# codeandkey/kami

Hardware: AMD Instinct MI355X
Metric: NN leaf-evals/sec at batch 512 (119×8×8 planes), 1/2/4/8 MI355X (higher is better)
Workload: dtype bf16

## Files before the change

kami_amd/csrc/tower8_mfma.hip:

```cpp
#include "tower_common.h"

#include <atomic>

namespace kh {

using f32x4_t = float __attribute__((ext_vector_type(4)));
__device__ __forceinline__ void store_wt(f32x4_t* p, f32x4_t v) { asm volatile("global_store_dwordx4 %0, %1, off sc1" ::"v"(p), "v"(v) : "memory"); }
__device__ __forceinline__ void store_wt(float* p, float v) { asm volatile("global_store_dword %0, %1, off sc1" ::"v"(p), "v"(v) : "memory"); }

constexpr int T8_LAG = 1;
struct CPipe { unsigned ring; int cslot; };

__device__ __forceinline__ unsigned cpipe_advance(CPipe& p)
{
    p.cslot = (p.cslot + 1 == RING_D) ? 0 : p.cslot + 1;
    return p.ring + p.cslot * CHUNK;
}

__device__ __forceinline__ unsigned cpipe_step(CPipe& p)
{
    asm volatile("s_barrier" ::: "memory");
    __builtin_amdgcn_sched_barrier(0);
    p.cslot = (p.cslot + 1 == RING_D) ? 0 : p.cslot + 1;
    return p.ring + p.cslot * CHUNK;
}

__device__ __forceinline__ void pipe_issue4(Pipe& p, int hw, int lane)
{
    const char* sbase = p.stream + (size_t)p.next * CHUNK + hw * 4096;
    const unsigned dst = p.ring + p.islot * CHUNK + hw * 4096;
    const unsigned voff = lane * 16;
    unsigned keep;
    asm volatile("s_mov_b32 %0, m0\n\ts_mov_b32 m0, %3\n\ts_nop 0\n\t"
                 "global_load_lds_dwordx4 %1, %2\n\tglobal_load_lds_dwordx4 %1, %2 offset:1024\n\t"
                 "global_load_lds_dwordx4 %1, %2 offset:2048\n\tglobal_load_lds_dwordx4 %1, %2 offset:3072\n\t"
                 "s_mov_b32 m0, %0"
                 : "=&s"(keep) : "v"(voff), "s"(sbase), "s"(dst) : "memory");
    p.next = (p.next + 1 == p.nch) ? 0 : p.next + 1;
    p.islot = (p.islot + 1 == RING_D) ? 0 : p.islot + 1;
}

template <int VMX>
__device__ __forceinline__ void hpipe_step(Pipe& p, int hw, int lane)
{
    asm volatile("s_waitcnt vmcnt(%0)" ::"n"(4 * (RING_D - 3 - T8_LAG) + VMX) : "memory");
    asm volatile("s_barrier" ::: "memory");
    pipe_issue4(p, hw, lane);
}

template <typename T, int TAPS, int KS, int MS, int PAR, int NREG = 0, bool CF = false, int TAILV = 0>
__device__ __forceinline__ void gemm8_layer(CPipe& p, const char* smem, int lane, unsigned b_base, int stride,
                                            f32x16 (&acc)[MS], typename Elem<T>::vec8 (&A)[2][8],
                                            const typename Elem<T>::vec8* breg = nullptr)
{
    using V = typename Elem<T>::vec8;
    using S = LayerShape<TAPS, KS, MS>;
    constexpr int KPC = S::KPC;
    constexpr int NF = KPC * MS;
    V B[2][KPC];
#pragma unroll
    for (int k = 0; k < KPC; ++k) {
        if (k < NREG) B[PAR][k] = breg[k];
        else B[PAR][k] = *reinterpret_cast<const V*>(smem + b_base + b_offset<TAPS, KS, CF>(k, stride));
    }
#pragma unroll
    for (int n = 0; n < S::NCH; ++n) {
        const int cur = (PAR + n) & 1, nxt = cur ^ 1;
        const unsigned a_off = cpipe_step(p) + lane * 16;
#pragma unroll
        for (int f = 0; f < 8; ++f)
            if (n + 1 == S::NCH || f < NF) A[nxt][f] = *reinterpret_cast<const V*>(smem + a_off + f * 1024);
        if (n + 1 < S::NCH) {
#pragma unroll
            for (int k = 0; k < KPC; ++k) {
                if ((n + 1) * KPC + k < NREG) B[nxt][k] = breg[(n + 1) * KPC + k];
                else B[nxt][k] = *reinterpret_cast<const V*>(smem + b_base + b_offset<TAPS, KS, CF>((n + 1) * KPC + k, stride));
            }
        }
        if (TAILV > 0 && n == S::NCH - 1) {
#pragma unroll
            for (int ms = 0; ms < MS; ++ms)
#pragma unroll
                for (int k = 0; k < KPC; ++k) acc[ms] = Elem<T>::mfma(A[cur][k * MS + ms], B[cur][k], acc[ms]);
#pragma unroll
            for (int i = 0; i < KPC; ++i) {
                __builtin_amdgcn_sched_group_barrier(0x100, 2, 0);
                __builtin_amdgcn_sched_group_barrier(0x008, 1, 0);
            }
#pragma unroll
            for (int i = 0; i < (MS - 1) * KPC; ++i) {
                __builtin_amdgcn_sched_group_barrier(0x008, 1, 0);
                if (i > 0) __builtin_amdgcn_sched_group_barrier(0x002, TAILV, 0);
            }
            continue;
        }
#pragma unroll
        for (int k = 0; k < KPC; ++k)
#pragma unroll
            for (int ms = 0; ms < MS; ++ms) acc[ms] = Elem<T>::mfma(A[cur][k * MS + ms], B[cur][k], acc[ms]);
#pragma unroll
        for (int i = 0; i < NF; ++i) {
            __builtin_amdgcn_sched_group_barrier(0x100, 2, 0);
            __builtin_amdgcn_sched_group_barrier(0x008, 1, 0);
        }
    }
}

template <typename T, int PAR>
__device__ __forceinline__ void gemm8_dummy(CPipe& p, const char* smem, int lane, typename Elem<T>::vec8 (&A)[2][8])
{
    using V = typename Elem<T>::vec8;
    const unsigned a_off = cpipe_step(p) + lane * 16;
#pragma unroll
    for (int f = 0; f < 8; ++f) A[PAR ^ 1][f] = *reinterpret_cast<const V*>(smem + a_off + f * 1024);
}


enum { BM_RASTER = 0, BM_CENTRE = 1, BM_QUARTERS = 2 };
template <int TAPS, int KS, int BM>
__device__ __forceinline__ constexpr unsigned b_off8(int kk, int stride)
{
    if constexpr (BM == BM_QUARTERS) {
        const int pass = kk / (TAPS * KS / 4), k = kk % (TAPS * KS / 4);
        return b_offset<TAPS, KS / 4, false>(k, stride) + pass * (KS / 4) * 32;
    }
    return b_offset<TAPS, KS, BM == BM_CENTRE>(kk, stride);
}

template <typename T, int TAPS, int KS, int MS, int PAR, int NREG, int BM, int N0, int N1, bool BARMID = false>
__device__ __forceinline__ void gemm8_steps(CPipe& p, const char* smem, int lane, unsigned b_base, int stride,
                                            f32x16 (&acc)[MS], typename Elem<T>::vec8 (&A)[2][8],
                                            typename Elem<T>::vec8 (&B)[2][8 / MS],
                                            const typename Elem<T>::vec8* breg = nullptr)
{
    using V = typename Elem<T>::vec8;
    using S = LayerShape<TAPS, KS, MS>;
    constexpr int KPC = S::KPC;
#pragma unroll
    for (int n = N0; n < N1; ++n) {
        const int cur = (PAR + n) & 1, nxt = cur ^ 1;
        if (BARMID && n == N0) {
            static_assert(!BARMID || (MS == 2 && KPC == 4), "mid-step barrier: 2 x 4 chunk");
            const unsigned a_off = cpipe_advance(p) + lane * 16;
#pragma unroll
            for (int k = 0; k < 2; ++k) {
#pragma unroll
                for (int ms = 0; ms < 2; ++ms) {
                    const int i = 2 * k + ms;
                    A[nxt][2 * i] = *reinterpret_cast<const V*>(smem + a_off + (2 * i) * 1024);
                    A[nxt][2 * i + 1] = *reinterpret_cast<const V*>(smem + a_off + (2 * i + 1) * 1024);
                    acc[ms] = Elem<T>::mfma(A[cur][k * MS + ms], B[cur][k], acc[ms]);
                    __builtin_amdgcn_sched_barrier(0);
                }
            }
            asm volatile("s_barrier" ::: "memory");
#pragma unroll
            for (int k = 2; k < 4; ++k) {
#pragma unroll
                for (int ms = 0; ms < 2; ++ms) {
                    if (k == 2 && n + 1 < S::NCH) {
#pragma unroll
                        for (int j = 0; j < 2; ++j) {
                            const int kk = 2 * ms + j;
                            if ((n + 1) * KPC + kk < NREG) B[nxt][kk] = breg[(n + 1) * KPC + kk];
                            else B[nxt][kk] = *reinterpret_cast<const V*>(smem + b_base + b_off8<TAPS, KS, BM>((n + 1) * KPC + kk, stride));
                        }
                    }
                    acc[ms] = Elem<T>::mfma(A[cur][k * MS + ms], B[cur][k], acc[ms]);
                    __builtin_amdgcn_sched_barrier(0);
                }
            }
            continue;
        }
        const unsigned a_off = cpipe_step(p) + lane * 16;
#pragma unroll
        for (int f = 0; f < 8; ++f) A[nxt][f] = *reinterpret_cast<const V*>(smem + a_off + f * 1024);
        if (n + 1 < S::NCH) {
#pragma unroll
            for (int k = 0; k < KPC; ++k) {
                if ((n + 1) * KPC + k < NREG) B[nxt][k] = breg[(n + 1) * KPC + k];
                else B[nxt][k] = *reinterpret_cast<const V*>(smem + b_base + b_off8<TAPS, KS, BM>((n + 1) * KPC + k, stride));
            }
        }
#pragma unroll
        for (int k = 0; k < KPC; ++k)
#pragma unroll
            for (int ms = 0; ms < MS; ++ms) acc[ms] = Elem<T>::mfma(A[cur][k * MS + ms], B[cur][k], acc[ms]);
#pragma unroll
        for (int i = 0; i < 8; ++i) {
            __builtin_amdgcn_sched_group_barrier(0x100, 2, 0);
            __builtin_amdgcn_sched_group_barrier(0x008, 1, 0);
        }
    }
}

enum { EPI_STEM = 0, EPI_PACK = 1, EPI_RESID = 2 };

template <typename T, int EPI, int G>
__device__ __forceinline__ u32x2 epi_group(const f32x16& acc, f32x16& xf)
{
    u32x2 o;
    if (EPI == EPI_PACK) {
        o.x = relu_pk(pack2<T>(acc[4 * G + 0], acc[4 * G + 1]));
        o.y = relu_pk(pack2<T>(acc[4 * G + 2], acc[4 * G + 3]));
    } else {
#pragma unroll
        for (int i = 0; i < 4; ++i) {
            const float t = relu_nan(acc[4 * G + i]);
            xf[4 * G + i] = EPI == EPI_RESID ? xf[4 * G + i] + t : t;
        }
        o.x = pack2<T>(xf[4 * G + 0], xf[4 * G + 1]);
        o.y = pack2<T>(xf[4 * G + 2], xf[4 * G + 3]);
    }
    return o;
}

#define T8_FENCE() __builtin_amdgcn_sched_barrier(0)

template <typename T, int EPI, int CURP>
__device__ __forceinline__ void boundary(CPipe& p, char* smem, int lane, f32x16 (&acc)[2], f32x16 (&nacc)[2],
                                         unsigned nshift, typename Elem<T>::vec8 (&A)[2][8],
                                         typename Elem<T>::vec8 (&B)[2][4], f32x16 (&xf)[2], unsigned out_pix, unsigned nb_base)
{
    using V = typename Elem<T>::vec8;
    constexpr int cur = CURP, nxt = CURP ^ 1;
    u32x2 o[2][4];
#define T8_LDN(ms, g) do { const float4 s_ = *reinterpret_cast<const float4*>(smem + nshift + ((ms) * 32 + 8 * (g)) * 4); \
        nacc[ms][4 * (g) + 0] = s_.x; nacc[ms][4 * (g) + 1] = s_.y; nacc[ms][4 * (g) + 2] = s_.z; nacc[ms][4 * (g) + 3] = s_.w; } while (0)
#define T8_ST(t, g) (*reinterpret_cast<u32x2*>(smem + out_pix + ((t) * 32 + 8 * (g)) * 2) = o[t][g])
#define T8_FRAG(ks) __builtin_bit_cast(V, (u32x4){ o[(ks) >> 1][2 * ((ks) & 1)].x, o[(ks) >> 1][2 * ((ks) & 1)].y, \
                                                   o[(ks) >> 1][2 * ((ks) & 1) + 1].x, o[(ks) >> 1][2 * ((ks) & 1) + 1].y })
    const unsigned a_off = cpipe_step(p) + lane * 16;
#define T8_RDA(set, f, off) (A[set][f] = *reinterpret_cast<const V*>(smem + (off) + (f) * 1024))
    T8_LDN(0, 0); T8_LDN(0, 1); acc[0] = Elem<T>::mfma(A[cur][0], B[cur][0], acc[0]); T8_FENCE();
    T8_LDN(0, 2); T8_LDN(0, 3); acc[0] = Elem<T>::mfma(A[cur][2], B[cur][1], acc[0]); T8_FENCE();
    T8_LDN(1, 0); T8_LDN(1, 1); acc[0] = Elem<T>::mfma(A[cur][4], B[cur][2], acc[0]); T8_FENCE();
    T8_LDN(1, 2); T8_LDN(1, 3); acc[0] = Elem<T>::mfma(A[cur][6], B[cur][3], acc[0]); T8_FENCE();
    T8_RDA(nxt, 0, a_off); T8_RDA(nxt, 1, a_off); acc[1] = Elem<T>::mfma(A[cur][1], B[cur][0], acc[1]); T8_FENCE();
    T8_RDA(nxt, 2, a_off); T8_RDA(nxt, 3, a_off); acc[1] = Elem<T>::mfma(A[cur][3], B[cur][1], acc[1]); T8_FENCE();
    T8_RDA(nxt, 4, a_off); T8_RDA(nxt, 5, a_off);
    o[0][0] = epi_group<T, EPI, 0>(acc[0], xf[0]); o[0][1] = epi_group<T, EPI, 1>(acc[0], xf[0]);
    acc[1] = Elem<T>::mfma(A[cur][5], B[cur][2], acc[1]); T8_FENCE();
    T8_RDA(nxt, 6, a_off); T8_RDA(nxt, 7, a_off);
    o[0][2] = epi_group<T, EPI, 2>(acc[0], xf[0]); o[0][3] = epi_group<T, EPI, 3>(acc[0], xf[0]);
    acc[1] = Elem<T>::mfma(A[cur][7], B[cur][3], acc[1]); T8_FENCE();
// ... 3 lines not shown
        T8_ST(0, 0); T8_ST(0, 1); T8_RDA(cur, 0, a2);
        nacc[0] = Elem<T>::mfma(A[nxt][0], f0, nacc[0]); T8_FENCE();
        T8_ST(0, 2); T8_ST(0, 3); T8_RDA(cur, 1, a2);
        nacc[1] = Elem<T>::mfma(A[nxt][1], f0, nacc[1]); T8_FENCE();
    }
    {
        const V f1 = T8_FRAG(1);
        T8_RDA(cur, 2, a2); T8_RDA(cur, 3, a2);
        nacc[0] = Elem<T>::mfma(A[nxt][2], f1, nacc[0]); T8_FENCE();
        T8_RDA(cur, 4, a2); T8_RDA(cur, 5, a2);
        o[1][0] = epi_group<T, EPI, 0>(acc[1], xf[1]); o[1][1] = epi_group<T, EPI, 1>(acc[1], xf[1]);
        nacc[1] = Elem<T>::mfma(A[nxt][3], f1, nacc[1]); T8_FENCE();
    }
    {
        const V f2 = T8_FRAG(2);
        o[1][2] = epi_group<T, EPI, 2>(acc[1], xf[1]); o[1][3] = epi_group<T, EPI, 3>(acc[1], xf[1]);
        T8_ST(1, 0); T8_ST(1, 1); T8_ST(1, 2); T8_ST(1, 3);
        nacc[0] = Elem<T>::mfma(A[nxt][4], f2, nacc[0]); T8_FENCE();
        T8_RDA(cur, 6, a2); T8_RDA(cur, 7, a2);
        nacc[1] = Elem<T>::mfma(A[nxt][5], f2, nacc[1]); T8_FENCE();
    }
    {
        const V f3 = T8_FRAG(3);
        asm volatile("s_waitcnt lgkmcnt(2)\n\ts_barrier" ::: "memory");
#pragma unroll
        for (int k = 0; k < 4; ++k) B[cur][k] = *reinterpret_cast<const V*>(smem + nb_base + b_offset<9, TW_CP / 16, true>(4 + k, XSTR));
        nacc[0] = Elem<T>::mfma(A[nxt][6], f3, nacc[0]); T8_FENCE();
        nacc[1] = Elem<T>::mfma(A[nxt][7], f3, nacc[1]); T8_FENCE();
    }
#undef T8_LDN
#undef T8_ST
}

template <typename T, int EPI, int CURP>
__device__ __forceinline__ void tower_tail(CPipe& p, const char* smem, int lane, f32x16 (&acc)[2], typename Elem<T>::vec8 (&A)[2][8],
                                           typename Elem<T>::vec8 (&B)[2][4], f32x16 (&xf)[2], Packed<2>& xk)
{
    using V = typename Elem<T>::vec8;
    constexpr int cur = CURP, nxt = CURP ^ 1;
    const unsigned a_off = cpipe_step(p) + lane * 16;
    T8_RDA(nxt, 0, a_off); T8_RDA(nxt, 1, a_off); acc[0] = Elem<T>::mfma(A[cur][0], B[cur][0], acc[0]); T8_FENCE();
    T8_RDA(nxt, 2, a_off); T8_RDA(nxt, 3, a_off); acc[0] = Elem<T>::mfma(A[cur][2], B[cur][1], acc[0]); T8_FENCE();
    T8_RDA(nxt, 4, a_off); T8_RDA(nxt, 5, a_off); acc[0] = Elem<T>::mfma(A[cur][4], B[cur][2], acc[0]); T8_FENCE();
    T8_RDA(nxt, 6, a_off); T8_RDA(nxt, 7, a_off); acc[0] = Elem<T>::mfma(A[cur][6], B[cur][3], acc[0]); T8_FENCE();
    acc[1] = Elem<T>::mfma(A[cur][1], B[cur][0], acc[1]); T8_FENCE();
    acc[1] = Elem<T>::mfma(A[cur][3], B[cur][1], acc[1]); T8_FENCE();
    xk.o[0][0] = epi_group<T, EPI, 0>(acc[0], xf[0]); xk.o[0][1] = epi_group<T, EPI, 1>(acc[0], xf[0]);
    acc[1] = Elem<T>::mfma(A[cur][5], B[cur][2], acc[1]); T8_FENCE();
    xk.o[0][2] = epi_group<T, EPI, 2>(acc[0], xf[0]); xk.o[0][3] = epi_group<T, EPI, 3>(acc[0], xf[0]);
    acc[1] = Elem<T>::mfma(A[cur][7], B[cur][3], acc[1]); T8_FENCE();
    xk.o[1][0] = epi_group<T, EPI, 0>(acc[1], xf[1]); xk.o[1][1] = epi_group<T, EPI, 1>(acc[1], xf[1]);
    xk.o[1][2] = epi_group<T, EPI, 2>(acc[1], xf[1]); xk.o[1][3] = epi_group<T, EPI, 3>(acc[1], xf[1]);
}
#undef T8_RDA

template <int STRIDE>
__device__ __forceinline__ void zero_halo(char* base, int board_bytes, int t)
{
    const u32x4 z = { 0, 0, 0, 0 };
    for (int i = t; i < TW_NB * NPIX; i += 256) {
        const int pp = i % NPIX, yy = pp / PITCH, xx = pp % PITCH;
        if (yy >= 1 && yy <= 8 && xx >= 1 && xx <= 8) continue;
        char* d = base + (i / NPIX) * board_bytes + pp * STRIDE;
#pragma unroll
        for (int k = 0; k < STRIDE / 16; ++k) *reinterpret_cast<u32x4*>(d + k * 16) = z;
    }
}

template <bool LEGAL>
__device__ __forceinline__ void helper_value_fc(const TowerArgs& a, const float* v64, int b0, int j, int lane)
{
    asm volatile("s_barrier" ::: "memory");
    unsigned voff = (unsigned)j * 16u;
    asm volatile("" : "+v"(voff));
    float4 fcw[16];
#pragma unroll
    for (int k = 0; k < 16; ++k)
        fcw[k] = *reinterpret_cast<const float4*>(reinterpret_cast<const char*>(a.fcw4) + (size_t)k * KH_VALUE_WIDTH * 16 + voff);
    const float fcbias = a.fcb[j];
    __builtin_amdgcn_sched_barrier(0);
    asm volatile("s_barrier" ::: "memory");
    float s[TW_NB];
#pragma unroll
    for (int bb = 0; bb < TW_NB; ++bb) s[bb] = 0.0f;
    static_assert(TW_NB == 2, "value FC: two boards per workgroup");
#pragma unroll
    for (int k = 0; k < 16; ++k) {
        const float* vb = v64 + (k & ~3) * 4;
        if ((k & 3) == 0) asm volatile("" : "+v"(vb), "+v"(s[0]), "+v"(s[1]));
        const float4 w = fcw[k];
#pragma unroll
        for (int bb = 0; bb < TW_NB; ++bb) {
            const float4 x = *reinterpret_cast<const float4*>(vb + bb * 64 + (k & 3) * 4);
            s[bb] = fmaf(x.x, w.x, s[bb]); s[bb] = fmaf(x.y, w.y, s[bb]);
            s[bb] = fmaf(x.z, w.z, s[bb]); s[bb] = fmaf(x.w, w.w, s[bb]);
        }
    }
    bool nan = false;
#pragma unroll
    for (int bb = 0; bb < TW_NB; ++bb) {
        if (b0 + bb < a.B) {
            const float r = tanhf(s[bb] + fcbias);
            nan |= (r != r);
            store_wt(a.vfull + (size_t)(b0 + bb) * KH_VALUE_WIDTH + j, r);
            if (LEGAL && j == 0) a.lg_values[b0 + bb] = r;
        }
    }
    if (__any(nan) && lane == 0) raise_flag<LEGAL>(a, 1);
}

template <typename T, int KS_STEM, bool LEGAL = false>
__global__ __launch_bounds__(512) void tower8_kernel(TowerArgs a)
{
    extern __shared__ __attribute__((aligned(16))) char smem[];
    constexpr int FP = KS_STEM * 16;
    constexpr int SSTR = FP * 2 + 16;
    constexpr int SBOARD = NPIX * SSTR;
    constexpr int ST_SIZE = st_size(FP);
    constexpr int LDS_PAR = LDS_ST + ST_SIZE;
    constexpr int LDS_L = LDS_X;
    using V = typename Elem<T>::vec8;
    constexpr int NSTEM = LayerShape<9, KS_STEM, 2>::NCH;
    constexpr int P1 = NSTEM & 1;
    constexpr int NLAYER = LayerShape<9, TW_CP / 16, 2>::NCH;
    constexpr int NPOL = LayerShape<1, TW_CP / 16, 4>::NCH + LayerShape<1, KH_POLICY_MID / 16, 3>::NCH + (P1 ? 1 : 0);

    const int tid = threadIdx.x;
    const int lane = tid & 63;
    const int wave = __builtin_amdgcn_readfirstlane(tid >> 6);
    const int ct = tid & 255;
    const int cw = wave & 3;
    const int R = a.R, F = a.F;

    float* par = reinterpret_cast<float*>(smem + LDS_PAR);
    const float* shift3 = par;
    const float* pshift1 = par + (1 + 2 * R) * TW_CP;
    const float* pbias2 = pshift1 + KH_POLICY_MID;
    const float* vw = pbias2 + 128;
    const float* vsh = vw + TW_CP;
    float* v64 = const_cast<float*>(vsh) + 4;
    float* red = v64 + TW_NB * 64;
    const int ngroups = (a.B + TW_NB - 1) / TW_NB;

    if (wave >= 6) {
        const int pt = tid & 127;
        for (int grp = blockIdx.x; grp < ngroups; grp += gridDim.x) {
            const int b0 = grp * TW_NB;
            if (KS_STEM == 8) {
                float4_u pl[4][8];
                const int lc = pt & 7;
                const int nb = min(TW_NB, a.B - b0);
                const char* gbase = reinterpret_cast<const char*>(a.in + (size_t)b0 * 64 * F);
                unsigned voff[8];
#pragma unroll
                for (int j = 0; j < 8; ++j) {
                    const int ip = (pt >> 3) + 16 * j;
                    voff[j] = (unsigned)((min(ip >> 6, nb - 1) * 64 + (ip & 63)) * F) * 4u;
                }
                const unsigned sdst = LDS_ST + ((((pt >> 6) + 1) * PITCH + ((pt >> 3) & 7) + 1) * SSTR) + 8 * lc;
                unsigned badmax = 0u;
                auto request = [&](int q) {
                    const unsigned cc = (unsigned)min(32 * q + 4 * lc, F - 4) * 4u;
#pragma unroll
                    for (int j = 0; j < 8; ++j)
                        pl[q][j] = __builtin_nontemporal_load(reinterpret_cast<const float4_u*>(gbase + voff[j] + cc));
                };
                auto convert = [&](int q, int j) {
                    float x[4] = { pl[q][j].x, pl[q][j].y, pl[q][j].z, pl[q][j].w };
                    if (32 * q + 32 > F) {
                        const int c = 32 * q + 4 * lc;
                        const int sh = c - min(c, F - 4);
                        float y[4];
#pragma unroll
                        for (int k = 0; k < 4; ++k) {
                            y[k] = sh == 0 ? x[k] : 0.0f;
#pragma unroll
                            for (int m = 1; m < 4; ++m)
                                if (k + m < 4) y[k] = sh == m ? x[k + m] : y[k];
                        }
#pragma unroll
                        for (int k = 0; k < 4; ++k) x[k] = y[k];
                    }
                    badmax = max(max(badmax, __float_as_uint(x[0]) & 0x7fffffffu), __float_as_uint(x[1]) & 0x7fffffffu);
                    badmax = max(max(badmax, __float_as_uint(x[2]) & 0x7fffffffu), __float_as_uint(x[3]) & 0x7fffffffu);
                    u32x2 o;
                    o.x = pack2<T>(x[0], x[1]); o.y = pack2<T>(x[2], x[3]);
                    *reinterpret_cast<u32x2*>(smem + sdst + (j >> 2) * SBOARD + (j & 3) * 2 * PITCH * SSTR + 64 * q) = o;
                };
                request(0); request(1); request(2); request(3);
#pragma unroll
                for (int j = 0; j < 8; ++j) convert(0, j);
                lds_barrier();
#pragma unroll
                for (int i = 0; i < NSTEM; ++i) {
                    if (i < 4) { convert(1, 2 * i); convert(1, 2 * i + 1); }
                    else if (i < 7) { convert(2, 2 * (i - 4)); convert(2, 2 * (i - 4) + 1); }
                    else if (i < 9) convert(2, i - 1);
                    else if (i < 13) { convert(3, 2 * (i - 9)); convert(3, 2 * (i - 9) + 1); }
                    if (i == 3 || i == 8 || i == 12) asm volatile("s_waitcnt lgkmcnt(0)" ::: "memory");
                    asm volatile("s_barrier" ::: "memory");
                }
                const bool bad = badmax >= 0x7f800000u;
                if (__any(bad) && lane == 0) raise_flag<LEGAL>(a, 0);
            } else {
                if (a.boards) {
                    const int bb = pt >> 6, p = pt & 63;
                    float v[32];
#pragma unroll
                    for (int k = 0; k < 32; ++k) v[k] = 0.0f;
                    if (b0 + bb < a.B) {
                        float w[KH_NFEATURES];
                        encode_square(a.boards + (b0 + bb), p, w);
#pragma unroll
                        for (int k = 0; k < KH_NFEATURES; ++k) v[k] = w[k];
                    }
                    char* dst = smem + LDS_ST + bb * SBOARD + (((p >> 3) + 1) * PITCH + (p & 7) + 1) * SSTR;
#pragma unroll
                    for (int c = 0; c < 4; ++c) {
                        u32x4 o;
                        o.x = pack2<T>(v[8 * c + 0], v[8 * c + 1]); o.y = pack2<T>(v[8 * c + 2], v[8 * c + 3]);
                        o.z = pack2<T>(v[8 * c + 4], v[8 * c + 5]); o.w = pack2<T>(v[8 * c + 6], v[8 * c + 7]);
                        *reinterpret_cast<u32x4*>(dst + c * 16) = o;
                    }
                } else {
                    constexpr int CH = FP / 8;
                    constexpr int NIT = TW_NB * 64 * CH / 128;
                    float vin[NIT][8];
                    const int c0 = (pt % CH) * 8;
#pragma unroll
                    for (int j = 0; j < NIT; ++j) {
                        const int i = pt + 128 * j;
                        const int bb = i / (64 * CH), p = (i / CH) & 63;
                        const float* src = a.in + ((size_t)(b0 + bb) * 64 + p) * F + c0;
                        const bool live = (b0 + bb) < a.B;
                        if (live && c0 + 8 <= F) {
                            const float4_u lo = *reinterpret_cast<const float4_u*>(src);
                            const float4_u hi = *reinterpret_cast<const float4_u*>(src + 4);
                            vin[j][0] = lo.x; vin[j][1] = lo.y; vin[j][2] = lo.z; vin[j][3] = lo.w;
                            vin[j][4] = hi.x; vin[j][5] = hi.y; vin[j][6] = hi.z; vin[j][7] = hi.w;
                        } else {
#pragma unroll
                            for (int k = 0; k < 8; ++k) vin[j][k] = (live && c0 + k < F) ? src[k] : 0.0f;
                        }
                    }
                    bool bad = false;
#pragma unroll
                    for (int j = 0; j < NIT; ++j) {
                        const int i = pt + 128 * j;
                        const int bb = i / (64 * CH), p = (i / CH) & 63;
                        u32x4 o;
                        unsigned w[4];
#pragma unroll
                        for (int k = 0; k < 4; ++k) {
                            const float lo = vin[j][2 * k], hi = vin[j][2 * k + 1];
                            bad = bad || !__builtin_isfinite(lo) || !__builtin_isfinite(hi);
                            w[k] = pack2<T>(lo, hi);
                        }
                        o.x = w[0]; o.y = w[1]; o.z = w[2]; o.w = w[3];
                        *reinterpret_cast<u32x4*>(smem + LDS_ST + bb * SBOARD + (((p >> 3) + 1) * PITCH + (p & 7) + 1) * SSTR + (pt % CH) * 16) = o;
                    }
                    if (__any(bad) && lane == 0) raise_flag<LEGAL>(a, 0);
                }
                lds_barrier();
                for (int i = 0; i < NSTEM; ++i) asm volatile("s_barrier" ::: "memory");
            }
            const int nsteps = 2 * R * NLAYER + NPOL;
            for (int i = 0; i < nsteps; ++i) {
                asm volatile("s_barrier" ::: "memory");
                if (i == 0 && R > 0) {
                    for (int z = 0; z < 2; ++z) zero_halo<XSTR>(smem + LDS_ST, XBOARD, pt + 128 * z);
                    asm volatile("s_waitcnt lgkmcnt(0)" ::: "memory");
                }
            }
            helper_value_fc<LEGAL>(a, v64, b0, tid & 255, lane);
            asm volatile("s_barrier" ::: "memory");
        }
    } else if (wave >= 4) {
        const int hw = wave - 4;
        const int nsteps = NSTEM + 2 * R * NLAYER + NPOL;
        Pipe pipe;
        pipe.stream = a.wstream; pipe.nch = a.nchunks; pipe.next = 0; pipe.islot = 0; pipe.ring = LDS_RING;
#pragma unroll
        for (int i = 0; i < RING_D - 1; ++i) pipe_issue4(pipe, hw, lane);

        for (int grp = blockIdx.x; grp < ngroups; grp += gridDim.x) {
            asm volatile("s_waitcnt vmcnt(%0)\n\ts_barrier" ::"n"(4 * (RING_D - 3)) : "memory");
            for (int i = 0; i < nsteps; ++i) hpipe_step<0>(pipe, hw, lane);
            helper_value_fc<LEGAL>(a, v64, grp * TW_NB, tid & 255, lane);
            asm volatile("s_barrier" ::: "memory");
        }
        asm volatile("s_waitcnt vmcnt(0)" ::: "memory");
    } else {
        const int h = lane >> 5;
        const int wb = cw >> 1;
        const int lp = PIXMAP[lane & 31];
        const int py = 4 * (cw & 1) + (lp >> 3), px = lp & 7;
        const unsigned xin = LDS_X + wb * XBOARD + (py * PITCH + px) * XSTR + h * 16;
        const unsigned tin = LDS_ST + wb * XBOARD + (py * PITCH + px) * XSTR + h * 16;
        const unsigned sin = LDS_ST + wb * SBOARD + (py * PITCH + px) * SSTR + h * 16;
        const unsigned xout = LDS_X + wb * XBOARD + ((py + 1) * PITCH + px + 1) * XSTR;
        const unsigned tout = LDS_ST + wb * XBOARD + ((py + 1) * PITCH + px + 1) * XSTR;
        unsigned xout_h = xout + 8 * h, tout_h = tout + 8 * h, sh0 = LDS_PAR + 16 * h;
        asm volatile("" : "+v"(xout_h), "+v"(tout_h), "+v"(sh0));

        CPipe pipe;
        pipe.ring = LDS_RING; pipe.cslot = 0;
        {
            const float4* src = reinterpret_cast<const float4*>(a.params);
            float4* dst = reinterpret_cast<float4*>(par);
            const int n4 = a.npar >> 2;
            for (int i0 = 0; i0 < n4; i0 += 4 * 256) {
                const float4 v0 = src[min(i0 + ct, n4 - 1)], v1 = src[min(i0 + 256 + ct, n4 - 1)];
                const float4 v2 = src[min(i0 + 512 + ct, n4 - 1)], v3 = src[min(i0 + 768 + ct, n4 - 1)];
                if (i0 + ct < n4) dst[i0 + ct] = v0;
                if (i0 + 256 + ct < n4) dst[i0 + 256 + ct] = v1;
                if (i0 + 512 + ct < n4) dst[i0 + 512 + ct] = v2;
                if (i0 + 768 + ct < n4) dst[i0 + 768 + ct] = v3;
            }
        }

        V A[2][8];
        bool first = true;

        for (int grp = blockIdx.x; grp < ngroups; grp += gridDim.x) {
            const int b0 = grp * TW_NB;
            zero_halo<XSTR>(smem + LDS_X, XBOARD, ct);
            zero_halo<SSTR>(smem + LDS_ST, SBOARD, ct);
            lds_barrier();
            if (first) {
                first = false;
#pragma unroll
                for (int f = 0; f < 8; ++f) A[0][f] = *reinterpret_cast<const V*>(smem + LDS_RING + lane * 16 + f * 1024);
            }

            Packed<2> xk;
            f32x16 xf[2];
#pragma unroll
            for (int i = 0; i < 16; ++i) { xf[0][i] = 0.0f; xf[1][i] = 0.0f; }
            f32x16 accA[2], accB[2];
            V B[2][4];
            acc_init<2>(accA, shift3, h);
            {
                constexpr int BMS = KS_STEM == 8 ? BM_QUARTERS : BM_RASTER;
#pragma unroll
                for (int k = 0; k < 4; ++k) B[0][k] = *reinterpret_cast<const V*>(smem + sin + b_off8<9, KS_STEM, BMS>(k, SSTR));
                gemm8_steps<T, 9, KS_STEM, 2, 0, 0, BMS, 0, NSTEM - 1>(pipe, smem, lane, sin, SSTR, accA, A, B);
            }
            constexpr int CP1 = P1 ^ 1;
            for (int r = 0; r < R; ++r) {
                boundary<T, EPI_RESID, CP1>(pipe, smem, lane, accA, accB, sh0 + (1 + 2 * r) * TW_CP * 4, A, B, xf, xout_h, xin);
                gemm8_steps<T, 9, TW_CP / 16, 2, P1, 4, BM_CENTRE, 1, 8, true>(pipe, smem, lane, xin, XSTR, accB, A, B);
                boundary<T, EPI_PACK, P1>(pipe, smem, lane, accB, accA, sh0 + (2 + 2 * r) * TW_CP * 4, A, B, xf, tout_h, tin);
                gemm8_steps<T, 9, TW_CP / 16, 2, P1 ^ 1, 4, BM_CENTRE, 1, 8, true>(pipe, smem, lane, tin, XSTR, accA, A, B);
            }
            tower_tail<T, EPI_RESID, CP1>(pipe, smem, lane, accA, A, B, xf, xk);

            {
                f32x2 s01 = { 0.0f, 0.0f }, s23 = { 0.0f, 0.0f };
#pragma unroll
                for (int ms = 0; ms < 2; ++ms)
#pragma unroll
                    for (int g = 0; g < 4; ++g) {
                        using f32x4 = float __attribute__((ext_vector_type(4)));
                        const f32x4 w = *reinterpret_cast<const f32x4*>(vw + ms * 32 + 8 * g + 4 * h);
                        const f32x2 x01 = { xf[ms][4 * g + 0], xf[ms][4 * g + 1] }, x23 = { xf[ms][4 * g + 2], xf[ms][4 * g + 3] };
                        s01 = x01 * w.xy + s01;
                        s23 = x23 * w.zw + s23;
                    }
                const float part = (s01.x + s01.y) + (s23.x + s23.y);
                const unsigned pu = __float_as_uint(part);
                if ((pu & 0x7f800000u) == 0x7f800000u) raise_flag<LEGAL>(a, 0);
                const auto sw = __builtin_amdgcn_permlane32_swap(pu, pu, false, false);
                const float sv = __uint_as_float(sw[0]) + __uint_as_float(sw[1]);
                if (h == 0) v64[wb * 64 + py * 8 + px] = relu_nan(sv + vsh[0]);
            }

            Packed<4> pk;
            {
                f32x16 acc[4];
                V bf[4];
                packed_fragments<T, 2>(xk, bf);
                acc_init<4>(acc, pshift1, h);
                asm volatile("s_waitcnt lgkmcnt(0)" ::: "memory");
                gemm8_layer<T, 1, TW_CP / 16, 4, P1, 4>(pipe, smem, lane, 0, 0, acc, A, bf);
                epilogue_pack<T, 4>(acc, pk);
            }
            {
                f32x16 acc[3];
                V bf[8];
                packed_fragments<T, 4>(pk, bf);
                acc_init<3>(acc, pbias2, h);
                gemm8_layer<T, 1, KH_POLICY_MID / 16, 3, P1, 8>(pipe, smem, lane, 0, 0, acc, A, bf);
                if (P1) gemm8_dummy<T, 1>(pipe, smem, lane, A);
                float* lrow = reinterpret_cast<float*>(smem + LDS_L + wb * LBOARD) + (py * 8 + px) * KH_POLICY_PLANES;
                float m = -INFINITY;
#pragma unroll
                for (int ms = 0; ms < 3; ++ms)
#pragma unroll
                    for (int g = 0; g < 4; ++g)
#pragma unroll
                        for (int i = 0; i < 4; ++i) {
                            const int plane = ms * 32 + 8 * g + 4 * h + i;
                            if (plane < KH_POLICY_PLANES) {
                                lrow[plane] = acc[ms][4 * g + i];
                                m = fmaxf(m, acc[ms][4 * g + i]);
                            }
                        }
                m = wave_max_f(m);
                if (lane == 0) red[cw] = m;
                lds_barrier();
            }

            {
                const int bb = ct >> 7, tt = ct & 127;
                const bool live = (b0 + bb) < a.B;
                const float4* L4 = reinterpret_cast<const float4*>(smem + LDS_L + bb * LBOARD);
                constexpr int NQ = KH_PSIZE / 4;
                float4 v[10];
#pragma unroll
                for (int k = 0; k < 10; ++k) {
                    const int q = tt + 128 * k;
                    v[k] = (q < NQ) ? L4[q] : make_float4(-INFINITY, -INFINITY, -INFINITY, -INFINITY);
                }
                const float m = fmaxf(red[bb * 2], red[bb * 2 + 1]);
                if (a.logits && live) {
                    float4* lo = reinterpret_cast<float4*>(a.logits + (size_t)(b0 + bb) * KH_PSIZE);
#pragma unroll
                    for (int k = 0; k < 10; ++k)
                        if (tt + 128 * k < NQ) lo[tt + 128 * k] = v[k];
                }
                float s = 0.0f;
#pragma unroll
                for (int k = 0; k < 10; ++k) {
                    v[k].x = __expf(v[k].x - m); v[k].y = __expf(v[k].y - m);
                    v[k].z = __expf(v[k].z - m); v[k].w = __expf(v[k].w - m);
                    s += (v[k].x + v[k].y) + (v[k].z + v[k].w);
                }
// ... 71 lines not shown
```

Measured before the change: 16.42 million.

## Overlap value-head sums with policy conv1 MFMAs and spread halo zeroing

Value-head weights are hoisted into registers, and the value dot product is interleaved into the first chunk of the policy conv1 GEMM through a side lambda with VALU scheduling groups. The explicit lgkmcnt wait before that GEMM is dropped. The helper waves now zero the T halo one piece per conv1 step, instead of doing the whole halo in one burst at step 0. The value FC store is vectorised: DPP gathers four lanes' outputs and one lane writes them as a dwordx4. Together these aim to hide VALU and LDS work behind MFMA latency, at the cost of added register pressure and more intricate ordering between the helper and compute waves.

```diff
diff --git a/kami_amd/csrc/tower8_mfma.hip b/kami_amd/csrc/tower8_mfma.hip
--- a/kami_amd/csrc/tower8_mfma.hip
+++ b/kami_amd/csrc/tower8_mfma.hip
@@ -1,6 +1,7 @@
 #include "tower_common.h"
 
 #include <atomic>
+
 
 namespace kh {
 
@@ -48,10 +49,10 @@
     pipe_issue4(p, hw, lane);
 }
 
-template <typename T, int TAPS, int KS, int MS, int PAR, int NREG = 0, bool CF = false, int TAILV = 0>
+template <typename T, int TAPS, int KS, int MS, int PAR, int NREG = 0, bool CF = false, int TAILV = 0, int SIDEV = 0, typename Side = int>
 __device__ __forceinline__ void gemm8_layer(CPipe& p, const char* smem, int lane, unsigned b_base, int stride,
                                             f32x16 (&acc)[MS], typename Elem<T>::vec8 (&A)[2][8],
-                                            const typename Elem<T>::vec8* breg = nullptr)
+                                            const typename Elem<T>::vec8* breg = nullptr, Side side = Side())
 {
     using V = typename Elem<T>::vec8;
     using S = LayerShape<TAPS, KS, MS>;
@@ -98,10 +99,12 @@
         for (int k = 0; k < KPC; ++k)
 #pragma unroll
             for (int ms = 0; ms < MS; ++ms) acc[ms] = Elem<T>::mfma(A[cur][k * MS + ms], B[cur][k], acc[ms]);
+        if constexpr (SIDEV > 0) if (n == 0) side();
 #pragma unroll
         for (int i = 0; i < NF; ++i) {
             __builtin_amdgcn_sched_group_barrier(0x100, 2, 0);
             __builtin_amdgcn_sched_group_barrier(0x008, 1, 0);
+            if (SIDEV > 0 && n == 0) __builtin_amdgcn_sched_group_barrier(0x002, SIDEV, 0);
         }
     }
 }
@@ -350,7 +353,11 @@
         if (b0 + bb < a.B) {
             const float r = tanhf(s[bb] + fcbias);
             nan |= (r != r);
-            store_wt(a.vfull + (size_t)(b0 + bb) * KH_VALUE_WIDTH + j, r);
+            const int ri = __float_as_int(r);
+            const f32x4_t q = { r, __int_as_float(__builtin_amdgcn_mov_dpp(ri, 0x55, 0xf, 0xf, true)),
+                                __int_as_float(__builtin_amdgcn_mov_dpp(ri, 0xaa, 0xf, 0xf, true)),
+                                __int_as_float(__builtin_amdgcn_mov_dpp(ri, 0xff, 0xf, 0xf, true)) };
+            if ((lane & 3) == 0) store_wt(reinterpret_cast<f32x4_t*>(a.vfull + (size_t)(b0 + bb) * KH_VALUE_WIDTH + j), q);
             if (LEGAL && j == 0) a.lg_values[b0 + bb] = r;
         }
     }
@@ -392,6 +399,11 @@
 
     if (wave >= 6) {
         const int pt = tid & 127;
+        constexpr int NHALO = NPIX - 64;
+        static_assert(TW_NB * NHALO <= 128 && XSTR == NLAYER * 16, "T halo: a pixel per plane-wave thread, a piece per conv1 step");
+        const int hq = pt % NHALO, hr = hq - 2 * PITCH;
+        const int hpp = hq < PITCH ? hq : hq < 2 * PITCH ? 9 * PITCH + hq - PITCH : (1 + (hr >> 2)) * PITCH + ((hr & 3) ? 8 + (hr & 3) : 0);
+        const unsigned thalo = LDS_ST + (pt / NHALO) * XBOARD + hpp * XSTR;
         for (int grp = blockIdx.x; grp < ngroups; grp += gridDim.x) {
             const int b0 = grp * TW_NB;
             if (KS_STEM == 8) {
@@ -513,13 +525,17 @@
                 for (int i = 0; i < NSTEM; ++i) asm volatile("s_barrier" ::: "memory");
             }
             const int nsteps = 2 * R * NLAYER + NPOL;
-            for (int i = 0; i < nsteps; ++i) {
-                asm volatile("s_barrier" ::: "memory");
-                if (i == 0 && R > 0) {
-                    for (int z = 0; z < 2; ++z) zero_halo<XSTR>(smem + LDS_ST, XBOARD, pt + 128 * z);
+            int i0 = 0;
+            if (R > 0) {
+#pragma unroll
+                for (int i = 0; i < NLAYER; ++i) {
+                    asm volatile("s_barrier" ::: "memory");
+                    if (pt < TW_NB * NHALO) *reinterpret_cast<u32x4*>(smem + thalo + 16 * i) = u32x4{ 0, 0, 0, 0 };
                     asm volatile("s_waitcnt lgkmcnt(0)" ::: "memory");
                 }
-            }
+                i0 = NLAYER;
+            }
+            for (int i = i0; i < nsteps; ++i) asm volatile("s_barrier" ::: "memory");
             helper_value_fc<LEGAL>(a, v64, b0, tid & 255, lane);
             asm volatile("s_barrier" ::: "memory");
         }
@@ -603,25 +619,33 @@
             }
             tower_tail<T, EPI_RESID, CP1>(pipe, smem, lane, accA, A, B, xf, xk);
 
-            {
+            using f32x4 = float __attribute__((ext_vector_type(4)));
+            f32x4 vwr[2][4];
+#pragma unroll
+            for (int ms = 0; ms < 2; ++ms)
+#pragma unroll
+                for (int g = 0; g < 4; ++g) vwr[ms][g] = *reinterpret_cast<const f32x4*>(vw + ms * 32 + 8 * g + 4 * h);
+            float part;
+            auto value_sums = [&]() {
                 f32x2 s01 = { 0.0f, 0.0f }, s23 = { 0.0f, 0.0f };
 #pragma unroll
                 for (int ms = 0; ms < 2; ++ms)
 #pragma unroll
                     for (int g = 0; g < 4; ++g) {
-                        using f32x4 = float __attribute__((ext_vector_type(4)));
-                        const f32x4 w = *reinterpret_cast<const f32x4*>(vw + ms * 32 + 8 * g + 4 * h);
+                        const f32x4 w = vwr[ms][g];
                         const f32x2 x01 = { xf[ms][4 * g + 0], xf[ms][4 * g + 1] }, x23 = { xf[ms][4 * g + 2], xf[ms][4 * g + 3] };
                         s01 = x01 * w.xy + s01;
                         s23 = x23 * w.zw + s23;
                     }
-                const float part = (s01.x + s01.y) + (s23.x + s23.y);
+                part = (s01.x + s01.y) + (s23.x + s23.y);
+            };
+            auto value_join = [&]() {
                 const unsigned pu = __float_as_uint(part);
                 if ((pu & 0x7f800000u) == 0x7f800000u) raise_flag<LEGAL>(a, 0);
                 const auto sw = __builtin_amdgcn_permlane32_swap(pu, pu, false, false);
                 const float sv = __uint_as_float(sw[0]) + __uint_as_float(sw[1]);
                 if (h == 0) v64[wb * 64 + py * 8 + px] = relu_nan(sv + vsh[0]);
-            }
+            };
 
             Packed<4> pk;
             {
@@ -629,8 +653,8 @@
                 V bf[4];
                 packed_fragments<T, 2>(xk, bf);
                 acc_init<4>(acc, pshift1, h);
-                asm volatile("s_waitcnt lgkmcnt(0)" ::: "memory");
-                gemm8_layer<T, 1, TW_CP / 16, 4, P1, 4>(pipe, smem, lane, 0, 0, acc, A, bf);
+                gemm8_layer<T, 1, TW_CP / 16, 4, P1, 4, false, 0, 3>(pipe, smem, lane, 0, 0, acc, A, bf, value_sums);
+                value_join();
                 epilogue_pack<T, 4>(acc, pk);
             }
             {
```

After: 16.44 million, median of 3. About the same (+0.1%).

## Interleave value head with policy conv MFMAs, spread halo zeroing, stop tail prefetch

Applied to the files above, without the earlier changes.

Merges the value-head dot product, its permlane reduction and the LDS store into the policy 1x1 conv's MFMA schedule so that VALU and LDS work overlaps matrix ops instead of running serially ahead of them. The helper wave's halo clearing is split into per-step pieces spread over the first conv steps, replacing a bulk zero pass that ran at step zero. The weight-stream waves now track how many steps remain, drain vmcnt progressively and stop issuing prefetches past the final step, which avoids wasted loads at the end. The risks are added bookkeeping and hand-scheduled code that must stay consistent with the ring depth and the barrier counts.

```diff
diff --git a/kami_amd/csrc/tower8_mfma.hip b/kami_amd/csrc/tower8_mfma.hip
--- a/kami_amd/csrc/tower8_mfma.hip
+++ b/kami_amd/csrc/tower8_mfma.hip
@@ -41,11 +41,13 @@
 }
 
 template <int VMX>
-__device__ __forceinline__ void hpipe_step(Pipe& p, int hw, int lane)
-{
-    asm volatile("s_waitcnt vmcnt(%0)" ::"n"(4 * (RING_D - 3 - T8_LAG) + VMX) : "memory");
+__device__ __forceinline__ void hpipe_step(Pipe& p, int hw, int lane, int left)
+{
+    if (left >= 0) asm volatile("s_waitcnt vmcnt(%0)" ::"n"(4 * (RING_D - 3 - T8_LAG) + VMX) : "memory");
+    else if (left == -1) asm volatile("s_waitcnt vmcnt(%0)" ::"n"(4 * (RING_D - 4 - T8_LAG) + VMX) : "memory");
+    else asm volatile("s_waitcnt vmcnt(%0)" ::"n"(VMX) : "memory");
     asm volatile("s_barrier" ::: "memory");
-    pipe_issue4(p, hw, lane);
+    if (left > 0) pipe_issue4(p, hw, lane);
 }
 
 template <typename T, int TAPS, int KS, int MS, int PAR, int NREG = 0, bool CF = false, int TAILV = 0>
@@ -300,6 +302,53 @@
     xk.o[1][0] = epi_group<T, EPI, 0>(acc[1], xf[1]); xk.o[1][1] = epi_group<T, EPI, 1>(acc[1], xf[1]);
     xk.o[1][2] = epi_group<T, EPI, 2>(acc[1], xf[1]); xk.o[1][3] = epi_group<T, EPI, 3>(acc[1], xf[1]);
 }
+
+template <typename T, int PAR>
+__device__ __forceinline__ bool policyconv_value(CPipe& p, char* smem, int lane, f32x16 (&acc)[4], typename Elem<T>::vec8 (&A)[2][8],
+                                                 const typename Elem<T>::vec8 (&bf)[4], const f32x16 (&xf)[2],
+                                                 unsigned vwh, unsigned vsh, unsigned v64p)
+{
+    using V = typename Elem<T>::vec8;
+    using f32x4 = float __attribute__((ext_vector_type(4)));
+    constexpr int cur = PAR, nxt = PAR ^ 1;
+    f32x2 s01 = { 0.0f, 0.0f }, s23 = { 0.0f, 0.0f };
+    f32x4 w[2][4];
+#define T8_VW(ms, g) (w[ms][g] = *reinterpret_cast<const f32x4*>(smem + vwh + ((ms) * 32 + 8 * (g)) * 4))
+#define T8_VF(ms, g) do { const f32x2 x01 = { xf[ms][4 * (g) + 0], xf[ms][4 * (g) + 1] }, x23 = { xf[ms][4 * (g) + 2], xf[ms][4 * (g) + 3] }; \
+        s01 = x01 * w[ms][g].xy + s01; s23 = x23 * w[ms][g].zw + s23; } while (0)
+#define T8_PM(set, n, k, ms) (acc[ms] = Elem<T>::mfma(A[set][(k) * 4 + (ms)], bf[2 * (n) + (k)], acc[ms]))
+    T8_VW(0, 0); T8_VW(0, 1); T8_VW(0, 2); T8_VW(0, 3);
+    const unsigned a1 = cpipe_step(p) + lane * 16;
+    T8_RDA(nxt, 0, a1); T8_RDA(nxt, 1, a1); T8_VW(1, 0); T8_VF(0, 0); T8_PM(cur, 0, 0, 0); T8_FENCE();
+    T8_RDA(nxt, 2, a1); T8_RDA(nxt, 3, a1); T8_VW(1, 1); T8_VF(0, 1); T8_PM(cur, 0, 0, 1); T8_FENCE();
+    T8_RDA(nxt, 4, a1); T8_RDA(nxt, 5, a1); T8_VW(1, 2); T8_VF(0, 2); T8_PM(cur, 0, 0, 2); T8_FENCE();
+    T8_RDA(nxt, 6, a1); T8_RDA(nxt, 7, a1); T8_VW(1, 3); T8_VF(0, 3); T8_PM(cur, 0, 0, 3); T8_FENCE();
+    const float shv = *reinterpret_cast<const float*>(smem + vsh);
+    T8_VF(1, 0); T8_PM(cur, 0, 1, 0); T8_FENCE();
+    T8_VF(1, 1); T8_PM(cur, 0, 1, 1); T8_FENCE();
+    T8_VF(1, 2); T8_PM(cur, 0, 1, 2); T8_FENCE();
+    T8_VF(1, 3); T8_PM(cur, 0, 1, 3); T8_FENCE();
+    const unsigned a2 = cpipe_step(p) + lane * 16;
+    const float part = (s01.x + s01.y) + (s23.x + s23.y);
+    const unsigned pu = __float_as_uint(part);
+    const bool bad = (pu & 0x7f800000u) == 0x7f800000u;
+    T8_RDA(cur, 0, a2); T8_RDA(cur, 1, a2); T8_PM(nxt, 1, 0, 0); T8_FENCE();
+    const auto sw = __builtin_amdgcn_permlane32_swap(pu, pu, false, false);
+    T8_RDA(cur, 2, a2); T8_RDA(cur, 3, a2); T8_PM(nxt, 1, 0, 1); T8_FENCE();
+    const float sv = __uint_as_float(sw[0]) + __uint_as_float(sw[1]);
+    const float vo = relu_nan(sv + shv);
+    T8_RDA(cur, 4, a2); T8_RDA(cur, 5, a2); T8_PM(nxt, 1, 0, 2); T8_FENCE();
+    *reinterpret_cast<float*>(smem + v64p) = vo;
+    T8_RDA(cur, 6, a2); T8_RDA(cur, 7, a2); T8_PM(nxt, 1, 0, 3); T8_FENCE();
+    T8_PM(nxt, 1, 1, 0); T8_FENCE();
+    T8_PM(nxt, 1, 1, 1); T8_FENCE();
+    T8_PM(nxt, 1, 1, 2); T8_FENCE();
+    T8_PM(nxt, 1, 1, 3); T8_FENCE();
+#undef T8_VW
+#undef T8_VF
+#undef T8_PM
+    return bad;
+}
 #undef T8_RDA
 
 template <int STRIDE>
@@ -313,6 +362,26 @@
 #pragma unroll
         for (int k = 0; k < STRIDE / 16; ++k) *reinterpret_cast<u32x4*>(d + k * 16) = z;
     }
+}
+
+constexpr int T_HALO_PIX = NPIX - 64;
+constexpr int T_HALO_PIECES = TW_NB * T_HALO_PIX * (XSTR / 16);
+constexpr int T_HALO_STEPS = (T_HALO_PIECES + 127) / 128;
+static_assert(T_HALO_STEPS < LayerShape<9, TW_CP / 16, 2>::NCH, "T's halo is cleared under conv1's steps in front of its epilogue");
+__device__ __forceinline__ void zero_halo_piece(char* base, int q)
+{
+    if (q >= T_HALO_PIECES) return;
+    const int hp = q / (XSTR / 16), k = q % (XSTR / 16);
+    const int bb = hp / T_HALO_PIX, j = hp % T_HALO_PIX;
+    int pp;
+    if (j < PITCH) pp = j;
+    else if (j < 2 * PITCH) pp = 9 * PITCH + (j - PITCH);
+    else {
+        const int jj = j - 2 * PITCH, c = jj & 3;
+        pp = (1 + (jj >> 2)) * PITCH + (c == 0 ? 0 : 8 + c);
+    }
+    const u32x4 z = { 0, 0, 0, 0 };
+    *reinterpret_cast<u32x4*>(base + bb * XBOARD + pp * XSTR + k * 16) = z;
 }
 
 template <bool LEGAL>
@@ -514,11 +583,9 @@
             }
             const int nsteps = 2 * R * NLAYER + NPOL;
             for (int i = 0; i < nsteps; ++i) {
+                if (i == NLAYER && R > 0) asm volatile("s_waitcnt lgkmcnt(0)" ::: "memory");
                 asm volatile("s_barrier" ::: "memory");
-                if (i == 0 && R > 0) {
-                    for (int z = 0; z < 2; ++z) zero_halo<XSTR>(smem + LDS_ST, XBOARD, pt + 128 * z);
-                    asm volatile("s_waitcnt lgkmcnt(0)" ::: "memory");
-                }
+                if (i < T_HALO_STEPS && R > 0) zero_halo_piece(smem + LDS_ST, i * 128 + pt);
             }
             helper_value_fc<LEGAL>(a, v64, b0, tid & 255, lane);
             asm volatile("s_barrier" ::: "memory");
@@ -530,10 +597,12 @@
         pipe.stream = a.wstream; pipe.nch = a.nchunks; pipe.next = 0; pipe.islot = 0; pipe.ring = LDS_RING;
 #pragma unroll
         for (int i = 0; i < RING_D - 1; ++i) pipe_issue4(pipe, hw, lane);
+        const int mygroups = (ngroups - (int)blockIdx.x + (int)gridDim.x - 1) / (int)gridDim.x;
+        int left = __builtin_amdgcn_readfirstlane(mygroups * nsteps - (RING_D - 1));
 
         for (int grp = blockIdx.x; grp < ngroups; grp += gridDim.x) {
             asm volatile("s_waitcnt vmcnt(%0)\n\ts_barrier" ::"n"(4 * (RING_D - 3)) : "memory");
-            for (int i = 0; i < nsteps; ++i) hpipe_step<0>(pipe, hw, lane);
+            for (int i = 0; i < nsteps; ++i, --left) hpipe_step<0>(pipe, hw, lane, left);
             helper_value_fc<LEGAL>(a, v64, grp * TW_NB, tid & 255, lane);
             asm volatile("s_barrier" ::: "memory");
         }
@@ -603,34 +672,17 @@
             }
             tower_tail<T, EPI_RESID, CP1>(pipe, smem, lane, accA, A, B, xf, xk);
 
-            {
-                f32x2 s01 = { 0.0f, 0.0f }, s23 = { 0.0f, 0.0f };
-#pragma unroll
-                for (int ms = 0; ms < 2; ++ms)
-#pragma unroll
-                    for (int g = 0; g < 4; ++g) {
-                        using f32x4 = float __attribute__((ext_vector_type(4)));
-                        const f32x4 w = *reinterpret_cast<const f32x4*>(vw + ms * 32 + 8 * g + 4 * h);
-                        const f32x2 x01 = { xf[ms][4 * g + 0], xf[ms][4 * g + 1] }, x23 = { xf[ms][4 * g + 2], xf[ms][4 * g + 3] };
-                        s01 = x01 * w.xy + s01;
-                        s23 = x23 * w.zw + s23;
-                    }
-                const float part = (s01.x + s01.y) + (s23.x + s23.y);
-                const unsigned pu = __float_as_uint(part);
-                if ((pu & 0x7f800000u) == 0x7f800000u) raise_flag<LEGAL>(a, 0);
-                const auto sw = __builtin_amdgcn_permlane32_swap(pu, pu, false, false);
-                const float sv = __uint_as_float(sw[0]) + __uint_as_float(sw[1]);
-                if (h == 0) v64[wb * 64 + py * 8 + px] = relu_nan(sv + vsh[0]);
-            }
-
             Packed<4> pk;
             {
                 f32x16 acc[4];
                 V bf[4];
                 packed_fragments<T, 2>(xk, bf);
                 acc_init<4>(acc, pshift1, h);
-                asm volatile("s_waitcnt lgkmcnt(0)" ::: "memory");
-                gemm8_layer<T, 1, TW_CP / 16, 4, P1, 4>(pipe, smem, lane, 0, 0, acc, A, bf);
+                const unsigned vw_h = (unsigned)(reinterpret_cast<const char*>(vw) - smem) + 16 * h;
+                const unsigned vsh_o = (unsigned)(reinterpret_cast<const char*>(vsh) - smem);
+                const unsigned v64_p = (unsigned)(reinterpret_cast<const char*>(v64) - smem) + (wb * 64 + py * 8 + px) * 4;
+                const bool bad = policyconv_value<T, P1>(pipe, smem, lane, acc, A, bf, xf, vw_h, vsh_o, v64_p);
+                if (bad) raise_flag<LEGAL>(a, 0);
                 epilogue_pack<T, 4>(acc, pk);
             }
             {
```

After: 16.66 million before, 16.29 million after. 0.978x the previous value.

## Interleave LDS reads with MFMAs, spread halo zeroing, and add a start-up barrier

Applied to the files above, without the earlier changes.

The GEMM step loops now issue A and B LDS reads interleaved per k-slice, and scheduling group barriers are spread evenly across the MFMAs through a new level_reads helper. The helper waves zero the T halo in eight slices across the first pipeline steps rather than all at once. A first-iteration barrier handshake between the DMA, helper and compute waves lets the compute waves read the first ring chunk only after it has landed. The aim is to smooth LDS traffic against the MFMA issue and trim start-up stalls. The risk is that the extra barriers, which must match across wave roles, could deadlock or add latency if miscounted.

```diff
diff --git a/kami_amd/csrc/tower8_mfma.hip b/kami_amd/csrc/tower8_mfma.hip
--- a/kami_amd/csrc/tower8_mfma.hip
+++ b/kami_amd/csrc/tower8_mfma.hip
@@ -9,6 +9,7 @@
 __device__ __forceinline__ void store_wt(float* p, float v) { asm volatile("global_store_dword %0, %1, off sc1" ::"v"(p), "v"(v) : "memory"); }
 
 constexpr int T8_LAG = 1;
+constexpr int T8_PIECES = 4;
 struct CPipe { unsigned ring; int cslot; };
 
 __device__ __forceinline__ unsigned cpipe_advance(CPipe& p)
@@ -31,11 +32,21 @@
     const unsigned dst = p.ring + p.islot * CHUNK + hw * 4096;
     const unsigned voff = lane * 16;
     unsigned keep;
+    static_assert(T8_PIECES == 4, "four 1 KB pieces per wave and chunk");
+#ifdef T8_DMA2
+    asm volatile("s_mov_b32 %0, m0\n\ts_mov_b32 m0, %3\n\ts_nop 0\n\t"
+                 "global_load_lds_dwordx4 %1, %2\n\tglobal_load_lds_dwordx4 %1, %2 offset:1024\n\t"
+                 "s_sleep 2\n\t"
+                 "global_load_lds_dwordx4 %1, %2 offset:2048\n\tglobal_load_lds_dwordx4 %1, %2 offset:3072\n\t"
+                 "s_mov_b32 m0, %0"
+                 : "=&s"(keep) : "v"(voff), "s"(sbase), "s"(dst) : "memory");
+#else
     asm volatile("s_mov_b32 %0, m0\n\ts_mov_b32 m0, %3\n\ts_nop 0\n\t"
                  "global_load_lds_dwordx4 %1, %2\n\tglobal_load_lds_dwordx4 %1, %2 offset:1024\n\t"
                  "global_load_lds_dwordx4 %1, %2 offset:2048\n\tglobal_load_lds_dwordx4 %1, %2 offset:3072\n\t"
                  "s_mov_b32 m0, %0"
                  : "=&s"(keep) : "v"(voff), "s"(sbase), "s"(dst) : "memory");
+#endif
     p.next = (p.next + 1 == p.nch) ? 0 : p.next + 1;
     p.islot = (p.islot + 1 == RING_D) ? 0 : p.islot + 1;
 }
@@ -43,9 +54,21 @@
 template <int VMX>
 __device__ __forceinline__ void hpipe_step(Pipe& p, int hw, int lane)
 {
-    asm volatile("s_waitcnt vmcnt(%0)" ::"n"(4 * (RING_D - 3 - T8_LAG) + VMX) : "memory");
+    asm volatile("s_waitcnt vmcnt(%0)" ::"n"(T8_PIECES * (RING_D - 3 - T8_LAG) + VMX) : "memory");
     asm volatile("s_barrier" ::: "memory");
     pipe_issue4(p, hw, lane);
+}
+
+__device__ __forceinline__ void level_reads(int nr, int ng)
+{
+#pragma unroll
+    for (int i = 0; i < 8; ++i) {
+        if (i >= ng) continue;
+        const int c = ((i + 1) * nr + ng - 1) / ng - (i * nr + ng - 1) / ng;
+        if (c >= 2) __builtin_amdgcn_sched_group_barrier(0x100, 2, 0);
+        else if (c == 1) __builtin_amdgcn_sched_group_barrier(0x100, 1, 0);
+        __builtin_amdgcn_sched_group_barrier(0x008, 1, 0);
+    }
 }
 
 template <typename T, int TAPS, int KS, int MS, int PAR, int NREG = 0, bool CF = false, int TAILV = 0>
@@ -67,15 +90,20 @@
     for (int n = 0; n < S::NCH; ++n) {
         const int cur = (PAR + n) & 1, nxt = cur ^ 1;
         const unsigned a_off = cpipe_step(p) + lane * 16;
-#pragma unroll
-        for (int f = 0; f < 8; ++f)
-            if (n + 1 == S::NCH || f < NF) A[nxt][f] = *reinterpret_cast<const V*>(smem + a_off + f * 1024);
+        int nrd = 0;
         if (n + 1 < S::NCH) {
 #pragma unroll
             for (int k = 0; k < KPC; ++k) {
+#pragma unroll
+                for (int ms = 0; ms < MS; ++ms) A[nxt][k * MS + ms] = *reinterpret_cast<const V*>(smem + a_off + (k * MS + ms) * 1024);
+                nrd += MS;
                 if ((n + 1) * KPC + k < NREG) B[nxt][k] = breg[(n + 1) * KPC + k];
-                else B[nxt][k] = *reinterpret_cast<const V*>(smem + b_base + b_offset<TAPS, KS, CF>((n + 1) * KPC + k, stride));
-            }
+                else { B[nxt][k] = *reinterpret_cast<const V*>(smem + b_base + b_offset<TAPS, KS, CF>((n + 1) * KPC + k, stride)); ++nrd; }
+            }
+        } else {
+#pragma unroll
+            for (int f = 0; f < 8; ++f) A[nxt][f] = *reinterpret_cast<const V*>(smem + a_off + f * 1024);
+            nrd = 8;
         }
         if (TAILV > 0 && n == S::NCH - 1) {
 #pragma unroll
@@ -98,11 +126,7 @@
         for (int k = 0; k < KPC; ++k)
 #pragma unroll
             for (int ms = 0; ms < MS; ++ms) acc[ms] = Elem<T>::mfma(A[cur][k * MS + ms], B[cur][k], acc[ms]);
-#pragma unroll
-        for (int i = 0; i < NF; ++i) {
-            __builtin_amdgcn_sched_group_barrier(0x100, 2, 0);
-            __builtin_amdgcn_sched_group_barrier(0x008, 1, 0);
-        }
+        level_reads(nrd, NF);
     }
 }
 
@@ -173,24 +197,21 @@
             continue;
         }
         const unsigned a_off = cpipe_step(p) + lane * 16;
-#pragma unroll
-        for (int f = 0; f < 8; ++f) A[nxt][f] = *reinterpret_cast<const V*>(smem + a_off + f * 1024);
-        if (n + 1 < S::NCH) {
-#pragma unroll
-            for (int k = 0; k < KPC; ++k) {
+        int nrd = 8;
+#pragma unroll
+        for (int k = 0; k < KPC; ++k) {
+#pragma unroll
+            for (int ms = 0; ms < MS; ++ms) A[nxt][k * MS + ms] = *reinterpret_cast<const V*>(smem + a_off + (k * MS + ms) * 1024);
+            if (n + 1 < S::NCH) {
                 if ((n + 1) * KPC + k < NREG) B[nxt][k] = breg[(n + 1) * KPC + k];
-                else B[nxt][k] = *reinterpret_cast<const V*>(smem + b_base + b_off8<TAPS, KS, BM>((n + 1) * KPC + k, stride));
+                else { B[nxt][k] = *reinterpret_cast<const V*>(smem + b_base + b_off8<TAPS, KS, BM>((n + 1) * KPC + k, stride)); ++nrd; }
             }
         }
 #pragma unroll
         for (int k = 0; k < KPC; ++k)
 #pragma unroll
             for (int ms = 0; ms < MS; ++ms) acc[ms] = Elem<T>::mfma(A[cur][k * MS + ms], B[cur][k], acc[ms]);
-#pragma unroll
-        for (int i = 0; i < 8; ++i) {
-            __builtin_amdgcn_sched_group_barrier(0x100, 2, 0);
-            __builtin_amdgcn_sched_group_barrier(0x008, 1, 0);
-        }
+        level_reads(nrd, 8);
     }
 }
 
@@ -315,6 +336,20 @@
     }
 }
 
+constexpr int HALO_PIX = NPIX - 64;
+constexpr int HALO_PIECES = TW_NB * HALO_PIX * (XSTR / 16);
+static_assert(HALO_PIECES <= 8 * 128, "T's halo: eight slices of the two plane waves");
+__device__ __forceinline__ void zero_halo_slice(char* base, int id)
+{
+    if (id >= HALO_PIECES) return;
+    const int hp = id / (XSTR / 16), piece = id % (XSTR / 16);
+    const int board = hp / HALO_PIX, k = hp % HALO_PIX;
+    const int e = k - 2 * PITCH;
+    const int pp = k < PITCH ? k : k < 2 * PITCH ? 9 * PITCH + (k - PITCH) : (e / 4 + 1) * PITCH + ((e & 3) == 0 ? 0 : 8 + (e & 3));
+    const u32x4 z = { 0, 0, 0, 0 };
+    *reinterpret_cast<u32x4*>(base + board * XBOARD + pp * XSTR + piece * 16) = z;
+}
+
 template <bool LEGAL>
 __device__ __forceinline__ void helper_value_fc(const TowerArgs& a, const float* v64, int b0, int j, int lane)
 {
@@ -392,8 +427,10 @@
 
     if (wave >= 6) {
         const int pt = tid & 127;
+        bool first = true;
         for (int grp = blockIdx.x; grp < ngroups; grp += gridDim.x) {
             const int b0 = grp * TW_NB;
+            if (KS_STEM != 8 && first) asm volatile("s_barrier" ::: "memory");
             if (KS_STEM == 8) {
                 float4_u pl[4][8];
                 const int lc = pt & 7;
@@ -435,7 +472,9 @@
                     o.x = pack2<T>(x[0], x[1]); o.y = pack2<T>(x[2], x[3]);
                     *reinterpret_cast<u32x2*>(smem + sdst + (j >> 2) * SBOARD + (j & 3) * 2 * PITCH * SSTR + 64 * q) = o;
                 };
-                request(0); request(1); request(2); request(3);
+                request(0); request(1);
+                if (first) asm volatile("s_barrier" ::: "memory");
+                request(2); request(3);
 #pragma unroll
                 for (int j = 0; j < 8; ++j) convert(0, j);
                 lds_barrier();
@@ -515,13 +554,14 @@
             const int nsteps = 2 * R * NLAYER + NPOL;
             for (int i = 0; i < nsteps; ++i) {
                 asm volatile("s_barrier" ::: "memory");
-                if (i == 0 && R > 0) {
-                    for (int z = 0; z < 2; ++z) zero_halo<XSTR>(smem + LDS_ST, XBOARD, pt + 128 * z);
-                    asm volatile("s_waitcnt lgkmcnt(0)" ::: "memory");
+                if (i < 8 && R > 0) {
+                    zero_halo_slice(smem + LDS_ST, i * 128 + pt);
+                    if (i == 7) asm volatile("s_waitcnt lgkmcnt(0)" ::: "memory");
                 }
             }
             helper_value_fc<LEGAL>(a, v64, b0, tid & 255, lane);
             asm volatile("s_barrier" ::: "memory");
+            first = false;
         }
     } else if (wave >= 4) {
         const int hw = wave - 4;
@@ -531,8 +571,9 @@
 #pragma unroll
         for (int i = 0; i < RING_D - 1; ++i) pipe_issue4(pipe, hw, lane);
 
+        if ((int)blockIdx.x < ngroups) asm volatile("s_waitcnt vmcnt(%0)\n\ts_barrier" ::"n"(T8_PIECES * (RING_D - 2)) : "memory");
         for (int grp = blockIdx.x; grp < ngroups; grp += gridDim.x) {
-            asm volatile("s_waitcnt vmcnt(%0)\n\ts_barrier" ::"n"(4 * (RING_D - 3)) : "memory");
+            asm volatile("s_waitcnt vmcnt(%0)\n\ts_barrier" ::"n"(T8_PIECES * (RING_D - 3)) : "memory");
             for (int i = 0; i < nsteps; ++i) hpipe_step<0>(pipe, hw, lane);
             helper_value_fc<LEGAL>(a, v64, grp * TW_NB, tid & 255, lane);
             asm volatile("s_barrier" ::: "memory");
@@ -572,22 +613,23 @@
 
         for (int grp = blockIdx.x; grp < ngroups; grp += gridDim.x) {
             const int b0 = grp * TW_NB;
+            if (first) {
+                first = false;
+                asm volatile("s_waitcnt lgkmcnt(0)\n\ts_barrier" ::: "memory");
+#pragma unroll
+                for (int f = 0; f < 8; ++f) A[0][f] = *reinterpret_cast<const V*>(smem + LDS_RING + lane * 16 + f * 1024);
+            }
+            f32x16 accA[2], accB[2];
+            acc_init<2>(accA, shift3, h);
             zero_halo<XSTR>(smem + LDS_X, XBOARD, ct);
             zero_halo<SSTR>(smem + LDS_ST, SBOARD, ct);
             lds_barrier();
-            if (first) {
-                first = false;
-#pragma unroll
-                for (int f = 0; f < 8; ++f) A[0][f] = *reinterpret_cast<const V*>(smem + LDS_RING + lane * 16 + f * 1024);
-            }
 
             Packed<2> xk;
             f32x16 xf[2];
 #pragma unroll
             for (int i = 0; i < 16; ++i) { xf[0][i] = 0.0f; xf[1][i] = 0.0f; }
-            f32x16 accA[2], accB[2];
             V B[2][4];
-            acc_init<2>(accA, shift3, h);
             {
                 constexpr int BMS = KS_STEM == 8 ? BM_QUARTERS : BM_RASTER;
 #pragma unroll
```

Result: slower. 16.77 million before, 16.51 million after (-1.6%).
